# alucas2/raytracing-potato

Measured on AMD Instinct MI355X. Metric: Mrays/s at 1920×1080×256spp bunny scene; 1/2/4/8-GPU scaling + %HBM roofline, higher is better.
Workload: dtype f64

## Files before the change

include/rp_host.h:

```cpp
#ifndef RP_HOST_H
#define RP_HOST_H

#include <stdint.h>

#include "rp.h"

#ifdef __cplusplus
extern "C" {
#endif

typedef struct rph_mesh {
  uint32_t n_vertices, n_indices;
  double* positions;
  double* normals;
  double* uvs;
  uint32_t* indices;
} rph_mesh;

int rph_obj_load(const char* path, rph_mesh* out);
void rph_mesh_free(rph_mesh* m);

int rph_tga_load(const char* path, uint32_t* width, uint32_t* height, uint8_t** rgba);
int rph_tga_save(const char* path, uint32_t width, uint32_t height, const uint8_t* rgba);
void rph_free(void* p);
// ... 28 lines not shown
  uint32_t grid;
  uint64_t n_queue, out_stride;
  uint32_t dv_units[2], dv_tiles_x[2], dv_chunk[2];
} rph_launch_plan;
int rph_plan_launch(uint32_t width, uint32_t height, uint32_t spp, uint32_t max_bounce, uint32_t tile_w, uint32_t tile_h,
                    uint32_t shard, uint32_t num_shards, uint32_t samples_per_stream, uint32_t shard_map, uint32_t n_frames,
                    uint32_t frame_order, uint32_t unit_queues, uint32_t queue_chunk, uint64_t lanes, rph_launch_plan* out);

int rph_draw_round(uint32_t kind, uint32_t ring_blocks, const uint32_t* ring_image, uint32_t pos, double out[3],
                   uint32_t* new_pos, uint32_t* accepted);

int rph_ray_setup(uint32_t node_format, double qbound, const double* rays, uint64_t n, float* out);

int rph_prim_test(uint32_t kind, const double g[9], const double* rays, uint64_t n, double* out);

const char* rph_last_error(void);

#ifdef __cplusplus
}
#endif
#endif
```

raytracing-potato_amd/csrc/rp_device.h:

```cpp
#pragma once
#include <hip/hip_runtime.h>

#include "rp_kernel.h"

#pragma clang fp contract(off)

#include "rp_draw.h"
#include "rp_ray.h"
#include "rp_isect.h"

#if defined(RPK_ABLATE_RNG) || defined(RPK_ABLATE_UV) || defined(RPK_ABLATE_TEX) || defined(RPK_ABLATE_METAL) || \
    defined(RPK_BATCH_LEAF)
#error "result-changing experiment macros are not part of the product kernel"
#endif
#if defined(RPK_NT_STORE) || defined(RPK_NT_ALL) || defined(RPK_NT_TEX) || defined(RPK_NT_OUT) ||           \
    defined(RPK_SLAB_ALIGN) || defined(RPK_SLAB_PAD) || defined(RPK_COLD_SLAB) || defined(RPK_COLD_IN_SLAB) || \
    defined(RPK_W3) || defined(RPK_W4) || defined(RPK_WAVES) || defined(RPK_TRIES_BALL) ||             \
    defined(RPK_NO_SPECULATIVE) || defined(RPK_NODE_BREAK) || defined(RPK_TRIES) || defined(RPK_RING) ||       \
    defined(RPK_RNG_BATCH) || defined(RPK_RNG_CRIT) || defined(RPK_PRIM_BREAK) || defined(RPK_PRIO_TRAV) ||    \
    defined(RPK_PRIO_SHADE) || defined(RPK_PRIO_REFILL) || defined(RPK_SORT_Q) || defined(RPK_WF_REFILL)
#error "experiment macros are not part of the product kernel (tools/build_variant.sh patches a copy instead)"
#endif

namespace rpk {
// ... 123 lines not shown
  }
  return make_uint4(o[0], o[1], o[2], o[3]);
}

RPK_INLINE void seed_key(uint64_t state, uint32_t key[8]) {
#pragma unroll
  for (int c = 0; c < 8; c++) {
    state = state * 6364136223846793005ull + 11634580027462260723ull;
    uint32_t xs = (uint32_t)(((state >> 18) ^ state) >> 27);
    uint32_t rot = (uint32_t)(state >> 59);
    key[c] = (xs >> rot) | (xs << ((32 - rot) & 31));
  }
}

static constexpr uint32_t RING = 8;
static constexpr uint32_t SLAB_KEY = 0, SLAB_RING = 2;
static constexpr uint32_t RNG_CRIT = 2, RNG_BATCH = 48;
static constexpr uint32_t PRIM_BREAK = 12;

template <uint32_t RN>
struct RngT {
  static constexpr uint32_t ring = RN;
  static constexpr uint32_t tail_n = rpd::ring_tail_words(RN) / 4;
  static constexpr uint32_t tail = SLAB_RING + 4 * RN, jit = tail + tail_n, lane_n = jit + 8;
  static_assert(RN > RNG_CRIT && RN <= RING && (RN & (RN - 1)) == 0,
                "ring: a power of two above the critical refill level (a full ring is never refilled), <= RING");
  static_assert(lane_n % 2 == 0, "lane slab stride must be a multiple of 32 B (keystream blocks on whole sectors)");
  uint4* slab;
  uint32_t pos;
  uint32_t* end;
  uint32_t* jtag;
};
template <class Rng>
RPK_INLINE void store_key(Rng& r, const uint32_t k[8]) {
  r.slab[SLAB_KEY] = make_uint4(k[0], k[1], k[2], k[3]);
  r.slab[SLAB_KEY + 1] = make_uint4(k[4], k[5], k[6], k[7]);
}
RPK_INLINE void store_block(uint4* dst, const uint32_t w[16]) {
#pragma unroll
  for (int q = 0; q < 4; q++) {
    dst[q] = make_uint4(w[4 * q], w[4 * q + 1], w[4 * q + 2], w[4 * q + 3]);
  }
}
RPK_INLINE void store_ring_block(uint4* dst, uint4* tail, const uint32_t w[16]) {
  store_block(dst, w);
  if (tail) {
#pragma unroll
    for (uint32_t q = 0; q < rpd::TAIL_WORDS / 4; q++) tail[q] = make_uint4(w[4 * q], w[4 * q + 1], w[4 * q + 2], w[4 * q + 3]);
  }
}
RPK_INLINE void load_block(const uint4* src, uint32_t w[16]) {
#pragma unroll
  for (int q = 0; q < 4; q++) {
    const uint4 v = src[q];
    w[4 * q] = v.x; w[4 * q + 1] = v.y; w[4 * q + 2] = v.z; w[4 * q + 3] = v.w;
  }
}
template <uint32_t RN>
RPK_INLINE uint4* ring_slot(const RngT<RN>& r, uint32_t b) { return r.slab + SLAB_RING + 4 * (b & (RN - 1u)); }
template <uint32_t RN>
RPK_INLINE uint4* ring_tail(uint4* slab, uint32_t b) {
  return RngT<RN>::tail_n != 0 && (b & (RN - 1u)) == 0u ? slab + RngT<RN>::tail : nullptr;
}
template <uint32_t RN>
RPK_INLINE uint4* jit_slot(const RngT<RN>& r, uint32_t b) { return r.slab + RngT<RN>::jit + 4 * (b & 1u); }

RPK_INLINE uint32_t nth_set(uint64_t m, uint32_t n) {
  uint32_t pos = 0;
#pragma unroll
  for (int w = 32; w >= 1; w >>= 1) {
    const uint32_t c = (uint32_t)__popcll(m & ((1ull << w) - 1ull));
    if (n >= c) { n -= c; m >>= w; pos += (uint32_t)w; }
  }
  return pos;
}
static_assert(BLOCK == 64, "rng_refill: a block is one wave, so a lane's slab is the wave's lane index past the first");
template <uint32_t RN>
RPK_INLINE void rng_refill(RngT<RN>& r, bool alive, bool fresh, uint64_t seed, uint32_t s, uint32_t spp) {
  const uint32_t cur = r.pos >> 4, end = *r.end, have = end - cur;
  const uint32_t b1 = (s + 1) >> 2, b2 = b1 + 1;
  const bool j1 = alive && !fresh && 4 * b1 < spp && r.jtag[(b1 & 1u) * BLOCK] != b1;
  const bool j2 = alive && !fresh && 4 * b2 < spp && r.jtag[(b2 & 1u) * BLOCK] != b2;
  const bool crit = alive && (fresh || have <= RNG_CRIT);
  const bool room = alive && (fresh || have < RN || j1 || j2);
  if (__ballot(crit) == 0 && (uint32_t)__popcll(__ballot(room)) < RNG_BATCH) return;
  const bool main = fresh || crit || !(j1 || j2);
  const uint32_t b = fresh ? 0u : (main ? end : (j1 ? b1 : b2));
  const uint32_t end1 = !room ? end : (fresh ? 1u : (main ? end + 1u : end));
  const uint32_t have1 = end1 - (fresh ? 0u : cur);
  const uint32_t want = alive && have1 <= RNG_CRIT ? min(RNG_CRIT + 1u - have1, RN - have1) : 0u;
  const uint64_t m1 = __ballot(want >= 1u), m2 = __ballot(want >= 2u), ex = __ballot(!room);
  const uint32_t lane = __lane_id();
  const uint64_t below = (1ull << lane) - 1ull;
  const uint32_t n1 = (uint32_t)__popcll(m1), nreq = n1 + (uint32_t)__popcll(m2), nex = (uint32_t)__popcll(ex);
  const uint32_t xr = (uint32_t)__popcll(ex & below);
  const bool sec = !room && xr < nreq;
  uint32_t owner = lane, j = 0u;
  if (sec) {
    if (xr < n1) owner = nth_set(m1, xr);
    else { owner = nth_set(m2, xr - n1); j = 1u; }
  }
  const uint32_t slo = __shfl((uint32_t)seed, (int)owner), shi = __shfl((uint32_t)(seed >> 32), (int)owner);
  const uint32_t oend = __shfl(end1, (int)owner);
  const uint32_t served = (uint32_t)(want >= 1u && (uint32_t)__popcll(m1 & below) < nex) +
                          (uint32_t)(want >= 2u && n1 + (uint32_t)__popcll(m2 & below) < nex);
  if (room || sec) {
    DREG(DREG_REFILL)
    uint32_t k[8], w[16];
    seed_key(room ? seed : ((uint64_t)shi << 32 | slo), k);
    if (fresh) {
      DREG(DREG_BEGIN_PIXEL)
      store_key(r, k);
    }
    const uint32_t bb = room ? b : oend + j;
    chacha12(k, bb, w);
    uint4* oslab = r.slab + ((int)owner - (int)lane) * (int)RngT<RN>::lane_n;
    uint4* dst = room && !main ? jit_slot(r, b) : oslab + SLAB_RING + 4u * (bb & (RN - 1u));
    store_ring_block(dst, room && !main ? nullptr : ring_tail<RN>(oslab, bb), w);
    if (fresh) store_block(jit_slot(r, 0), w);
  }
  if (room) {
    if (fresh) {
      r.pos = 0;
      r.jtag[0] = 0;
      r.jtag[BLOCK] = 0xFFFFFFFFu;
    } else if (!main) {
      r.jtag[(b & 1u) * BLOCK] = b;
    }
  }
  if (room || served) *r.end = end1 + served;
  __builtin_amdgcn_fence(__ATOMIC_ACQ_REL, "wavefront");
}

static __device__ __attribute__((noinline, unused)) void gen_block(const uint4* slab, uint32_t b, uint4* dst, uint4* tail) {
  const uint4 a = slab[SLAB_KEY], c = slab[SLAB_KEY + 1];
  const uint32_t k[8] = {a.x, a.y, a.z, a.w, c.x, c.y, c.z, c.w};
  uint32_t w[16];
  chacha12(k, b, w);
  store_ring_block(dst, tail, w);
}

template <uint32_t RN>
RPK_INLINE uint4 rng_jitter(RngT<RN>& r, uint32_t s) {
  const uint32_t b = s >> 2;
  if (r.jtag[(b & 1u) * BLOCK] != b) {
    DREG(DREG_JIT_FALLBACK)
    gen_block(r.slab, b, jit_slot(r, b), nullptr);
    r.jtag[(b & 1u) * BLOCK] = b;
  }
  return jit_slot(r, b)[s & 3u];
}

using rpd::TRIES;
static_assert((RING & (RING - 1)) == 0, "the ring is indexed as 16 * ring words (a power of two)");
typedef uint32_t u32x4_a8 __attribute__((ext_vector_type(4), aligned(8)));
template <uint32_t STRIDE, uint32_t RN>
RPK_INLINE void ring_window(const RngT<RN>& r, uint32_t a, rpd::Try& t) {
  t.w[4] = 0; t.w[5] = 0;
  if constexpr (RngT<RN>::tail_n != 0) {
    const char* p = reinterpret_cast<const char*>(r.slab + SLAB_RING) + 4u * rpd::value_word(a, 0, RN);
    const u32x4_a8 v = *reinterpret_cast<const u32x4_a8*>(p);
    t.w[0] = v.x; t.w[1] = v.y; t.w[2] = v.z; t.w[3] = v.w;
    if (STRIDE == 6u) {
      const uint2 z = *reinterpret_cast<const uint2*>(p + 16);
      t.w[4] = z.x; t.w[5] = z.y;
    }
  } else {
    const uint2* ring = reinterpret_cast<const uint2*>(r.slab + SLAB_RING);
#pragma unroll
    for (uint32_t k = 0; k < STRIDE / 2u; k++) {
      const uint2 v = ring[rpd::value_word(a, k, RN) >> 1];
      t.w[2 * k] = v.x; t.w[2 * k + 1] = v.y;
    }
  }
}
template <uint32_t RN>
RPK_INLINE void ring_ensure(RngT<RN>& r, uint32_t last_blk) {
  while (last_blk >= *r.end) {
    DREG(DREG_RNG_FALLBACK)
    const uint32_t b = *r.end;
    gen_block(r.slab, b, ring_slot(r, b), ring_tail<RN>(r.slab, b));
    *r.end = b + 1;
  }
}
template <uint32_t STRIDE, uint32_t RN>
RPK_INLINE bool ring_round(RngT<RN>& r, uint32_t a, rpd::Draw& q) {
  ring_ensure(r, rpd::round_last_block(a, STRIDE));
  rpd::Try t[TRIES];
#pragma unroll
  for (uint32_t j = 0; j < TRIES; j++) ring_window<STRIDE>(r, a + STRIDE * j, t[j]);
  return rpd::draw_pick(STRIDE, a, t, q, r.pos);
}
template <uint32_t RN>
RPK_INLINE double gen_f64(RngT<RN>& r) {
  ring_ensure(r, r.pos >> 4);
  const uint2 v = reinterpret_cast<const uint2*>(r.slab + SLAB_RING)[rpd::window_word(r.pos, RN) >> 1];
  r.pos += 2;
  return rpd::words_unit(v.x, v.y);
}


typedef rpi::V3 V3;
RPK_INLINE V3 v3(double x, double y, double z) { V3 r; r.x = x; r.y = y; r.z = z; return r; }
RPK_INLINE V3 add(V3 a, V3 b) { return v3(a.x + b.x, a.y + b.y, a.z + b.z); }
RPK_INLINE V3 sub(V3 a, V3 b) { return v3(a.x - b.x, a.y - b.y, a.z - b.z); }
RPK_INLINE V3 mulc(V3 a, V3 b) { return v3(a.x * b.x, a.y * b.y, a.z * b.z); }
RPK_INLINE V3 smul(double s, V3 a) { return v3(s * a.x, s * a.y, s * a.z); }
RPK_INLINE double dot(V3 a, V3 b) { return (a.x * b.x + a.y * b.y) + a.z * b.z; }
RPK_INLINE double norm2(V3 a) { return (a.x * a.x + a.y * a.y) + a.z * a.z; }
RPK_INLINE V3 normalize(V3 a) { double n = sqrt(norm2(a)); return v3(a.x / n, a.y / n, a.z / n); }
RPK_INLINE V3 reflect(V3 i, V3 n) { return sub(i, smul(2.0 * dot(i, n), n)); }
// ... 127 lines not shown
    asm volatile("" : : "v"(g45.x), "v"(g45.y), "v"(g67.x), "v"(g67.y), "v"(g8k.x));
    rpi::sphere_test(g0, g23.y, o, d, tmin, best, [&](double t) {
      best = t; ts.bestp = (int32_t)k; ts.bestm = mat;
    });
  }
}

template <uint32_t NF>
RPK_INLINE void trav_begin(const KScene& S, V3 o, V3 d, double tmin, double tmax, TravState& t) {
  trav_init<NF>(S, tmax, t, d);
  double best = t.best;
  for (uint32_t k = S.always_first; k < S.always_first + S.n_always; k++) prim_test(S, k, o, d, tmin, best, t);
  t.best = best;
}

typedef __attribute__((address_space(3))) uint32_t lds_u32;
typedef __attribute__((address_space(1))) uint32_t glb_u32;
RPK_INLINE glb_u32* spill_ptr(const KScene& S) { return (glb_u32*)S.spill; }
template <bool SPILL>
RPK_INLINE void stk_put(const KScene& S, lds_u32* stk, uint32_t stride, uint32_t spl, uint32_t i, uint32_t v) {
  if (!SPILL || i < S.lds_depth) stk[i * stride] = v;
  else spill_ptr(S)[spl + i - S.lds_depth] = v;
}
template <bool SPILL>
RPK_INLINE uint32_t stk_get(const KScene& S, const lds_u32* stk, uint32_t stride, uint32_t spl, uint32_t i) {
  if (!SPILL || i < S.lds_depth) return stk[i * stride];
  return spill_ptr(S)[spl + i - S.lds_depth];
}

enum : uint32_t { WORK_VISIT = 2, WORK_TEST = 3, WORK_RAY = 16 };

// ... 804 lines not shown
```

raytracing-potato_amd/csrc/rp_host.cpp:

```cpp
#include "../../include/rp_host.h"

#include <algorithm>
#include <cmath>
#include <cstdio>
#include <cstdlib>
#include <cstring>
#include <fstream>
#include <string>
#include <thread>
#include <unordered_map>
#include <vector>

#include "rp_bvh.h"
#include "rp_draw.h"
#include "rp_isect.h"
#include "rp_kernel.h"
#include "rp_ray.h"
#include "rp_schedule.h"

namespace {

thread_local std::string g_err;

int fail(const std::string& m) {
  g_err = m;
  return RP_EINVAL;
}


struct Cursor {
  const char* p;
};
// ... 649 lines not shown

int rph_prim_test(uint32_t kind, const double g[9], const double* rays, uint64_t n, double* out) {
  if ((kind != rpl::PRIM_SPHERE && kind != rpl::PRIM_TRIANGLE) || !g || (n && (!rays || !out)))
    return fail("rph_prim_test: kind 0 (sphere) or 1 (triangle), non-NULL pointers");
  for (uint64_t r = 0; r < n; r++) {
    const double* q = rays + 8 * r;
    double* h = out + 4 * r;
    h[0] = h[1] = h[2] = h[3] = 0.0;
    prim_test(kind, g, {q[0], q[1], q[2]}, {q[3], q[4], q[5]}, q[6], q[7], [&](double t, double u, double v) {
      h[0] = 1.0; h[1] = t; h[2] = u; h[3] = v;
    });
  }
  return RP_OK;
}

int rph_draw_round(uint32_t kind, uint32_t ring_blocks, const uint32_t* ring_image, uint32_t pos, double out[3],
                   uint32_t* new_pos, uint32_t* accepted) {
  if (kind < rpd::DRAW_SPHERE || kind > rpd::DRAW_DISK || (ring_blocks != 4 && ring_blocks != 8) || (pos & 1u) ||
      !ring_image || !out || !new_pos || !accepted)
    return fail("rph_draw_round: kind 1-4, ring_blocks 4 or 8, even pos, non-NULL pointers");
  out[0] = out[1] = out[2] = 0.0;
  if (kind == rpd::DRAW_UNIFORM) {
    const uint32_t* p = ring_image + rpd::window_word(pos, ring_blocks);
    out[0] = rpd::words_unit(p[0], p[1]);
    *new_pos = pos + 2u;
    *accepted = 1u;
    return RP_OK;
  }
  const uint32_t stride = rpd::draw_stride(kind);
  rpd::Try t[rpd::TRIES];
// ... 78 lines not shown
```

raytracing-potato_amd/csrc/rp_kernel.h:

```cpp
#pragma once
#include <stdint.h>

#include "rp_layout.h"

namespace rpk {

struct KScene {
  const void* nodes;
  const rpl::Prim* prims;
  const rpl::PrimRef* prim_refs;
  const double* vnrm;
  const double* vuv;
  const rpl::Material* mats;
  const rpl::Texture* texs;
  const uint32_t* texels;
  rpl::Emit background;
  uint32_t root;
  uint32_t always_first, n_always;
  double qbound;
  uint32_t node_format;
  uint32_t leaf_break;
  uint32_t stack_depth;
  uint32_t lds_depth;
  uint64_t* diag;
  uint32_t* rng_slab;
  uint32_t* spill;
  uint32_t* unit_t0;
};

uint64_t rng_slab_bytes_per_lane(uint32_t node_format);
enum { RENDER_BLOCK = 64 };

enum { DIAG_N = 416, DIAG_DUR = 352, DIAG_DUR_N = 24, DIAG_DUR_LOG0 = 10 };
enum { DIAG_CYC = 320 };
enum {
  DCYC_SURF, DCYC_SPHUV, DCYC_TEXISSUE, DCYC_SCATTER, DCYC_TEXVAL, DCYC_EMIT, DCYC_START_SAMPLE, DCYC_END_SAMPLE,
  DCYC_NEWRAY, DCYC_REFILL, DCYC_NEXT_BOUNCE, DCYC_NODE_LOOP, DCYC_PRIM_LOOP, DCYC_N
};
#ifndef RPK_DIAG_BIN_TICKS
#define RPK_DIAG_BIN_TICKS 1000000
#endif
enum { DIAG_HIST = 64, DIAG_BIN_TICKS = RPK_DIAG_BIN_TICKS };
enum {
  DREG_NODE, DREG_PRIM, DREG_STEP, DREG_SHADE, DREG_SURF, DREG_SPHUV, DREG_TEX, DREG_LAMBERT, DREG_METAL,
  DREG_DIELEC, DREG_LOOP_LAMBERT, DREG_LOOP_METAL, DREG_END_SAMPLE, DREG_END_PIXEL, DREG_START_SAMPLE,
// ... 108 lines not shown
```

raytracing-potato_amd/csrc/rp_kernel.hip:

```cpp
#include "rp_device.h"

#pragma clang fp contract(off)

namespace rpk {

#define RPK_RENDER_ATTR __attribute__((amdgpu_waves_per_eu(4)))
static constexpr int PRIO_TRAV = 2, PRIO_SHADE = 1, PRIO_REFILL = 0;
template <uint32_t NF>
constexpr uint32_t RingFor = NF == rpl::NODES_Q8 ? 4u : RING;

RPK_INLINE bool meas_unit(uint32_t pipj, uint32_t batch) { return ((pipj ^ (pipj >> 16) ^ batch ^ (pipj >> 3)) & 7u) == 0u; }

template <bool PROBE, bool SPILL, uint32_t NF>
__global__ void __launch_bounds__(BLOCK) RPK_RENDER_ATTR render_kernel(const KArgs args) {
  extern __shared__ uint32_t lds_stack[];
  __shared__ unsigned long long blk_ctr[3];
  DIAG(__shared__ unsigned long long wmax[BLOCK / 64][8];
       if (threadIdx.x < BLOCK / 64 * 8) wmax[threadIdx.x / 8][threadIdx.x % 8] = 0;)
  if (threadIdx.x < 3) blk_ctr[threadIdx.x] = 0;
  DIAG(if (threadIdx.x < 2 * DREG_N) g_dreg[threadIdx.x] = 0;)
  DIAG(if (threadIdx.x < DCYC_N) g_dcyc[threadIdx.x] = 0;)
  DIAG(if (!PROBE && threadIdx.x == 0) atomicMax(&kargs()->diag[10], ~(unsigned long long)__builtin_amdgcn_s_memrealtime());)
  __syncthreads();
  lds_u32* stk = (lds_u32*)(lds_stack + threadIdx.x);

  uint64_t n_rays = 0, n_samples = 0, n_pixels = 0;
  DIAG(uint32_t lane_rays = 0;)
  bool overflow = false;
  DIAG(uint64_t ph[5] = {0, 0, 0, 0, 0}; uint64_t iters = 0, active = 0; TravDiag td; uint64_t t_prev = stamp();)
  DIAG(const uint64_t t_blk = __builtin_amdgcn_s_memrealtime(); uint64_t t_pix = t_blk, t_retire = t_blk; uint32_t rays_pix = 0;
       auto tbin = [&](uint64_t t) { return (uint32_t)min<uint64_t>((t - t_blk) / DIAG_BIN_TICKS, DIAG_HIST - 1); };)

  __shared__ double c_sum[3 * BLOCK];
  __shared__ double c_T[3 * BLOCK];
  __shared__ uint32_t c_u[8 * BLOCK];
  const uint32_t tid = threadIdx.x;
  uint32_t& slot = c_u[tid];
  uint32_t& pipj = c_u[BLOCK + tid];
  uint32_t& s = c_u[3 * BLOCK + tid];
  uint32_t& hits = c_u[4 * BLOCK + tid];
  uint32_t& batch = c_u[2 * BLOCK + tid];
  double& sum_x = c_sum[tid];
  double& sum_y = c_sum[BLOCK + tid];
  double& sum_z = c_sum[2 * BLOCK + tid];
  double& T_x = c_T[tid];
  double& T_y = c_T[BLOCK + tid];
  double& T_z = c_T[2 * BLOCK + tid];
  uint32_t depth = 0;
  uint32_t work = 0;
  bool first = true;
  RngT<RingFor<NF>> rng;
  rng.slab = reinterpret_cast<uint4*>(kargs()->S.rng_slab) + ((uint64_t)blockIdx.x * BLOCK + tid) * RngT<RingFor<NF>>::lane_n;
  rng.end = c_u + 5 * BLOCK + tid;
  rng.jtag = c_u + 6 * BLOCK + tid;
  rng.pos = 0;
  V3 o = v3(0, 0, 0), d = v3(0, 0, 1);
  T_x = T_y = T_z = 1.0;
  s = 0;
  hits = 0;
  sum_x = sum_y = sum_z = 0.0;
  TravState ts;
  ts.cur = rpl::ENTRY_EMPTY;
  ts.leaf = 0u;
  ts.sp = 0u;
  ts.best = 0.0;
  ts.bestp = -1;
  ts.bestm = KM_UNKNOWN;
  ts.bu = ts.bv = 0.0;
  ts.gy = ts.py = 0u;
// ... 566 lines not shown
  if (pos >= n) return;
  const uint32_t r = pos % N, k = pos / N, t = plan ? plan[pos] : pos;
  fcost[t] = sum[r * rank_stride + k];
  fcost[TILE_SORT_MAX + t] = mx[r * rank_stride + k];
}

int launch_learn_costs(const uint32_t* sum, const uint32_t* max, uint32_t rank_stride, uint32_t nranks, uint32_t n_tiles,
                       const uint32_t* plan, uint32_t* fcost, void* stream) {
  if (n_tiles == 0 || n_tiles > TILE_SORT_MAX || nranks == 0) return (int)hipErrorInvalidValue;
  hipLaunchKernelGGL(learn_costs_kernel, dim3((n_tiles + 255) / 256), dim3(256), 0, (hipStream_t)stream, sum, max,
                     rank_stride, nranks, n_tiles, plan, fcost);
  return (int)hipGetLastError();
}

uint64_t rng_slab_bytes_per_lane(uint32_t nf) {
  const uint32_t n = nf == rpl::NODES_Q8   ? RngT<RingFor<rpl::NODES_Q8>>::lane_n
                     : nf == rpl::NODES_W8 ? RngT<RingFor<rpl::NODES_W8>>::lane_n
                                           : RngT<RingFor<rpl::NODES_F32>>::lane_n;
  return (uint64_t)n * sizeof(uint4);
}

int render_blocks_per_cu(uint32_t lds_depth, bool spill, uint32_t nf, int* blocks) {
  const size_t lds = (size_t)lds_depth * BLOCK * sizeof(uint32_t);
  if (nf == rpl::NODES_W8) {
    if (spill) return (int)hipOccupancyMaxActiveBlocksPerMultiprocessor(blocks, render_kernel<false, true, rpl::NODES_W8>, BLOCK, lds);
    return (int)hipOccupancyMaxActiveBlocksPerMultiprocessor(blocks, render_kernel<false, false, rpl::NODES_W8>, BLOCK, lds);
  }
  if (nf == rpl::NODES_Q8) {
    if (spill) return (int)hipOccupancyMaxActiveBlocksPerMultiprocessor(blocks, render_kernel<false, true, rpl::NODES_Q8>, BLOCK, lds);
    return (int)hipOccupancyMaxActiveBlocksPerMultiprocessor(blocks, render_kernel<false, false, rpl::NODES_Q8>, BLOCK, lds);
  }
  if (spill) return (int)hipOccupancyMaxActiveBlocksPerMultiprocessor(blocks, render_kernel<false, true, rpl::NODES_F32>, BLOCK, lds);
  return (int)hipOccupancyMaxActiveBlocksPerMultiprocessor(blocks, render_kernel<false, false, rpl::NODES_F32>, BLOCK, lds);
}
// ... 20 lines not shown
```

raytracing-potato_amd/csrc/rp_scene.cpp:

```cpp
#include <chrono>
#include <cmath>

#include "rp_bvh.h"
#include "rp_state.h"

static_assert(rpk::CTR_N == RP_COUNTERS_LEN, "kernel counter block = the ABI's");
static_assert(rpk::CTR_RAYS == RP_CTR_RAYS && rpk::CTR_STATUS == RP_CTR_STATUS, "counter order");
static_assert(rpk::STATUS_STACK_OVERFLOW == RP_STATUS_STACK_OVERFLOW && rpk::STATUS_PLAN_MISMATCH == RP_STATUS_PLAN_MISMATCH,
              "status bits");
static_assert(sizeof(rp_render_params) == 48, "rp_render_params layout (bindings mirror it)");

__attribute__((visibility("hidden"))) thread_local std::string g_err;

namespace {

template <class T, class U>
int upload(const std::vector<T>& v, DevBuf<U>& out) {
  hipError_t e;
  if (!out.alloc((v.empty() ? 1 : v.size()) * (sizeof(T) / sizeof(U)), &e))
    return fail(RP_ENOMEM, std::string("hipMalloc: ") + hipGetErrorString(e));
  if (!v.empty()) {
    e = hipMemcpy(out.get(), v.data(), sizeof(T) * v.size(), hipMemcpyHostToDevice);
    if (e != hipSuccess) return fail(RP_EHIP, std::string("hipMemcpy: ") + hipGetErrorString(e));
  }
// ... 193 lines not shown
    return rc;
  if (!s->d_diag.alloc(rpk::DIAG_N) || hipMemset(s->d_diag.get(), 0, sizeof(uint64_t) * rpk::DIAG_N) != hipSuccess)
    return fail(RP_ENOMEM, "hipMalloc diagnostics");
  s->ks.diag = s->d_diag.get();
  s->ks.nodes = s->d_nodes.get(), s->ks.prims = s->d_prims.get(), s->ks.prim_refs = s->d_prim_refs.get();
  s->ks.vnrm = s->d_vnrm.get(), s->ks.vuv = s->d_vuv.get();
  s->ks.mats = s->d_mats.get(), s->ks.texs = s->d_texs.get(), s->ks.texels = s->d_texels.get();
  s->ks.background = ps.background;
  s->ks.root = ps.root;
  s->ks.always_first = ps.always_first;
  s->ks.n_always = ps.n_always;
  s->ks.qbound = ps.qbound;
  s->ks.node_format = node_format;
  s->ks.stack_depth = 3 * ps.max_depth + 4 + 3;
  if (node_format == rpl::NODES_W8) s->ks.stack_depth = 4 * (ps.max_depth + 1) + 3;
  if (s->ks.stack_depth < 17) s->ks.stack_depth = 17;
  const bool debug_stack = opt.debug_stack_depth != 0;
  if (debug_stack) s->ks.stack_depth = opt.debug_stack_depth;
  s->n_nodes = n_tree_nodes;
  s->n_leaves = ps.n_leaves;
  s->n_prims = desc->n_hittables;
  s->max_depth = ps.max_depth;
  s->device_bytes = rp_node_bytes(node_format) * n_tree_nodes + (sizeof(rpl::Prim) + sizeof(rpl::PrimRef)) * n_tree_prims +
                    sizeof(double) * 5 * n_vert + sizeof(rpl::Material) * ps.materials.size() +
                    sizeof(rpl::Texture) * ps.textures.size() + sizeof(uint32_t) * ps.texels.size();
  s->tiles_auto = RP_TILES_COST;
  s->ks.leaf_break = opt.leaf_break ? opt.leaf_break : (s->device_bytes > (256ull << 20) ? 16u : 8u);
  if (s->opt.trav_threshold == 0) s->opt.trav_threshold = s->device_bytes > (256ull << 20) ? 32u : DEF_TRAV_THRESHOLD;
  s->ks.lds_depth = s->ks.stack_depth;
  int bpc = 0;
  if (rpk::render_blocks_per_cu(s->ks.stack_depth, false, node_format, &bpc) != 0 || bpc < 1) bpc = 1;
  int bpc_spill = 0;
  if (!debug_stack && rpk::render_blocks_per_cu(17, true, node_format, &bpc_spill) == 0 && bpc_spill > bpc) {
    uint32_t L = s->ks.stack_depth - 1;
    int b = 0;
    while (L > 17 && (rpk::render_blocks_per_cu(L, true, node_format, &b) != 0 || b < bpc_spill)) L--;
    s->ks.lds_depth = L;
    bpc = bpc_spill;
  }
  if (!debug_stack && opt.lds_depth && opt.lds_depth < s->ks.stack_depth) {
    s->ks.lds_depth = opt.lds_depth;
    if (rpk::render_blocks_per_cu(opt.lds_depth, true, node_format, &bpc) != 0 || bpc < 1) bpc = 1;
  }
  s->blocks_per_cu = bpc;
  phase[4] = lap();
  if ((rc = ws_alloc(s.get(), &s->ws0))) return rc;
  phase[5] = lap();
  std::memcpy(s->build_s, phase, sizeof phase);
  *out = s.release();
  return RP_OK;
}
// ... 95 lines not shown
```

raytracing-potato_amd/rtpotato/_ffi.py:

```python
from __future__ import annotations

import ctypes
import os
from ctypes import (POINTER, Structure, c_char_p, c_double, c_float, c_int, c_int64, c_uint8, c_uint32,
                    c_uint64, c_void_p)

PKG_DIR = os.path.dirname(os.path.dirname(os.path.abspath(__file__)))
LIB_DIR = os.path.join(PKG_DIR, "lib")

RP_OK, RP_EINVAL, RP_EHIP, RP_ENOMEM, RP_ENODEV, RP_EINTERNAL, RP_ERCCL = 0, -1, -2, -3, -4, -5, -6
RP_HITTABLE_SPHERE, RP_HITTABLE_TRIANGLE = 0, 1
RP_SCATTER_NONE, RP_SCATTER_LAMBERT, RP_SCATTER_METAL, RP_SCATTER_DIELECTRIC = 0, 1, 2, 3
RP_ABSORB_BLACK_BODY, RP_ABSORB_WHITE_BODY, RP_ABSORB_ALBEDO, RP_ABSORB_ALBEDO_MAP = 0, 1, 2, 3
(RP_EMIT_NONE, RP_EMIT_DEBUG_NORMALS, RP_EMIT_COLOR, RP_EMIT_SKY_GRADIENT, RP_EMIT_SKY_SPHERE) = range(5)
(RP_TEXTURE_MISSING, RP_TEXTURE_DEBUG_UVS, RP_TEXTURE_SOLID, RP_TEXTURE_IMAGE, RP_TEXTURE_CHECKER,
 RP_TEXTURE_NOISE, RP_TEXTURE_PERLIN) = range(7)
RP_ROOT_BVH, RP_ROOT_LIST = 0, 1
RP_COUNTERS_LEN = 4
RP_SAMPLES_PER_STREAM = 32
RP_COMM_ID_BYTES = 128
RP_BUILDER_AUTO, RP_BUILDER_HOST, RP_BUILDER_DEVICE, RP_BUILDER_PLOC = 0, 1, 2, 3
RP_NODES_AUTO, RP_NODES_F32, RP_NODES_Q8, RP_NODES_W8 = 0, 1, 2, 3
RP_TILES_AUTO, RP_TILES_PLAIN, RP_TILES_COST, RP_TILES_MORTON, RP_TILES_PROBE = 0, 1, 2, 3, 4
RP_QUEUES_AUTO, RP_QUEUES_SINGLE, RP_QUEUES_XCD_TILES, RP_QUEUES_XCD_REGIONS = 0, 1, 2, 3
# ... 102 lines not shown
              "rp_render_multi", "rp_shard_unpack_map", "rp_workspace_tile_map", "rp_frame_assemble_ws", "rp_build_id",
              "rp_workspace_tile_costs", "rp_workspace_set_tile_costs", "rp_scene_build_times",
              "rp_workspace_frame_info", "rp_workspace_reserve_frames", "rp_render_frames_device_ws", "rp_frames_gather",
              "rp_workspace_unit_order", "rp_frames_block_words", "rp_frames_pack", "rp_frames_unpack",
              "rp_render_aov_device_ws", "rp_render_aov"]
class rph_launch_plan(Structure):
    _fields_ = [("n_shard_tiles", c_uint32), ("nbatch", c_uint32), ("plan_block", c_uint32), ("n_slots", c_uint64),
                ("gather_stride", c_uint64), ("block_words", c_uint64), ("queue_groups", c_uint32),
                ("queue_chunk", c_uint32), ("frames_inter", c_uint32), ("sortable", c_uint32), ("measure", c_uint32),
                ("grid", c_uint32), ("n_queue", c_uint64), ("out_stride", c_uint64), ("dv_units", c_uint32 * 2),
                ("dv_tiles_x", c_uint32 * 2), ("dv_chunk", c_uint32 * 2)]


HOST_SYMBOLS = ["rph_obj_load", "rph_mesh_free", "rph_tga_load", "rph_tga_save", "rph_free", "rph_to_srgb_u8",
                "rph_lookat", "rph_sky_panorama", "rph_bvh_selfcheck", "rph_bvh_traversal_stats", "rph_bvh_selfcheck_ex", "rph_bvh_traversal_stats_ex", "rph_bvh_tree_hash", "rph_last_error",
                "rph_stdrng_u64", "rph_make_div32", "rph_plan_launch", "rph_draw_round", "rph_ray_setup", "rph_prim_test"]


def rp_lib_path() -> str:
    return os.path.join(LIB_DIR, "librp.so")


def host_lib_path() -> str:
    return os.path.join(LIB_DIR, "librp_host.so")


def rp() -> ctypes.CDLL:
    global _rp
    if _rp is not None:
        return _rp
    path = os.environ.get("RP_LIB") or rp_lib_path()
# ... 98 lines not shown
    lib.rph_lookat.argtypes = [c_double * 3, c_double * 3, c_double * 3, c_double * 9]
    lib.rph_lookat.restype = None
    lib.rph_sky_panorama.argtypes = [c_uint32, c_uint32, c_void_p]
    lib.rph_bvh_selfcheck.argtypes = [POINTER(rp_scene_desc), c_uint32, POINTER(c_uint64)]
    lib.rph_bvh_traversal_stats.argtypes = [POINTER(rp_scene_desc), c_void_p, c_uint64, c_uint32, c_void_p]
    lib.rph_bvh_selfcheck_ex.argtypes = [POINTER(rp_scene_desc), c_uint32, c_uint32, POINTER(c_uint64)]
    lib.rph_bvh_traversal_stats_ex.argtypes = [POINTER(rp_scene_desc), c_void_p, c_uint64, c_uint32, c_uint32, c_void_p]
    lib.rph_bvh_tree_hash.argtypes = [POINTER(rp_scene_desc), c_uint32, c_uint32, POINTER(c_uint64)]
    lib.rph_last_error.restype = c_char_p
    lib.rph_stdrng_u64.argtypes = [c_void_p, c_uint64, c_uint64, c_void_p]
    lib.rph_make_div32.argtypes = [c_uint32, POINTER(c_uint32), POINTER(c_uint32)]
    lib.rph_draw_round.argtypes = [c_uint32, c_uint32, c_void_p, c_uint32, c_void_p, POINTER(c_uint32),
                                   POINTER(c_uint32)]
    lib.rph_ray_setup.argtypes = [c_uint32, c_double, c_void_p, c_uint64, c_void_p]
    lib.rph_prim_test.argtypes = [c_uint32, c_void_p, c_void_p, c_uint64, c_void_p]
    lib.rph_plan_launch.argtypes = [c_uint32] * 14 + [c_uint64, POINTER(rph_launch_plan)]
    _host = lib
    return lib


def check(code: int, lib: ctypes.CDLL | None = None) -> None:
    if code != RP_OK:
        lib = lib or rp()
        fn = lib.rp_last_error if hasattr(lib, "rp_last_error") else lib.rph_last_error
        raise RPError(code, (fn() or b"").decode(errors="replace"))


def check_host(code: int) -> None:
    if code != RP_OK:
        raise RPError(code, (host().rph_last_error() or b"").decode(errors="replace"))
# ... 4 lines not shown
```

Baseline: 7654.

## Keep per-lane ChaCha keys in LDS and route refill owners through LDS table

For non-Q8 node formats, each lane's ChaCha key is computed once per pixel and kept in shared memory instead of the global RNG slab. Secondary lanes that refill on another lane's behalf now read the owner's key from LDS rather than shuffling its seed and re-running seed_key. The owner-to-executor mapping is built through an LDS request table instead of the nth_set bit search. The RNG slab per lane shrinks by 32 B and the stack-depth LDS floor is lowered to offset the extra shared arrays. The cost is about 2.1 KB more LDS per block, which could lower occupancy or shrink the LDS traversal stack.

Result: no change. 7690 (median of 6 runs) (+0.5%).

```diff
diff --git a/include/rp_host.h b/include/rp_host.h
--- a/include/rp_host.h
+++ b/include/rp_host.h
@@ -66,6 +66,9 @@
 
 int rph_prim_test(uint32_t kind, const double g[9], const double* rays, uint64_t n, double* out);
 
+int rph_refill_assign(const uint8_t room[64], const uint8_t want[64], uint32_t owner[64], uint32_t block[64],
+                      uint32_t served[64]);
+
 const char* rph_last_error(void);
 
 #ifdef __cplusplus
diff --git a/raytracing-potato_amd/csrc/rp_device.h b/raytracing-potato_amd/csrc/rp_device.h
--- a/raytracing-potato_amd/csrc/rp_device.h
+++ b/raytracing-potato_amd/csrc/rp_device.h
@@ -6,6 +6,7 @@
 #pragma clang fp contract(off)
 
 #include "rp_draw.h"
+#include "rp_refill.h"
 #include "rp_ray.h"
 #include "rp_isect.h"
 
@@ -161,15 +162,18 @@
 }
 
 static constexpr uint32_t RING = 8;
-static constexpr uint32_t SLAB_KEY = 0, SLAB_RING = 2;
+typedef __attribute__((address_space(3))) uint32_t lds_u32;
+typedef __attribute__((address_space(3))) uint8_t lds_u8;
 static constexpr uint32_t RNG_CRIT = 2, RNG_BATCH = 48;
 static constexpr uint32_t PRIM_BREAK = 12;
 
-template <uint32_t RN>
+template <uint32_t RN, bool KL>
 struct RngT {
   static constexpr uint32_t ring = RN;
+  static constexpr bool key_lds = KL;
+  static constexpr uint32_t ring0 = KL ? 0u : 2u;
   static constexpr uint32_t tail_n = rpd::ring_tail_words(RN) / 4;
-  static constexpr uint32_t tail = SLAB_RING + 4 * RN, jit = tail + tail_n, lane_n = jit + 8;
+  static constexpr uint32_t tail = ring0 + 4 * RN, jit = tail + tail_n, lane_n = jit + 8;
   static_assert(RN > RNG_CRIT && RN <= RING && (RN & (RN - 1)) == 0,
                 "ring: a power of two above the critical refill level (a full ring is never refilled), <= RING");
   static_assert(lane_n % 2 == 0, "lane slab stride must be a multiple of 32 B (keystream blocks on whole sectors)");
@@ -177,11 +181,12 @@
   uint32_t pos;
   uint32_t* end;
   uint32_t* jtag;
+  lds_u32* key;
+  lds_u8* req;
 };
-template <class Rng>
-RPK_INLINE void store_key(Rng& r, const uint32_t k[8]) {
-  r.slab[SLAB_KEY] = make_uint4(k[0], k[1], k[2], k[3]);
-  r.slab[SLAB_KEY + 1] = make_uint4(k[4], k[5], k[6], k[7]);
+RPK_INLINE void load_key(const lds_u32* col, uint32_t k[8]) {
+#pragma unroll
+  for (int w = 0; w < 8; w++) k[w] = col[w * BLOCK];
 }
 RPK_INLINE void store_block(uint4* dst, const uint32_t w[16]) {
 #pragma unroll
@@ -203,27 +208,19 @@
     w[4 * q] = v.x; w[4 * q + 1] = v.y; w[4 * q + 2] = v.z; w[4 * q + 3] = v.w;
   }
 }
-template <uint32_t RN>
-RPK_INLINE uint4* ring_slot(const RngT<RN>& r, uint32_t b) { return r.slab + SLAB_RING + 4 * (b & (RN - 1u)); }
-template <uint32_t RN>
+template <uint32_t RN, bool KL>
+RPK_INLINE uint4* ring_slot(const RngT<RN, KL>& r, uint32_t b) { return r.slab + RngT<RN, KL>::ring0 + 4 * (b & (RN - 1u)); }
+template <uint32_t RN, bool KL>
 RPK_INLINE uint4* ring_tail(uint4* slab, uint32_t b) {
-  return RngT<RN>::tail_n != 0 && (b & (RN - 1u)) == 0u ? slab + RngT<RN>::tail : nullptr;
-}
-template <uint32_t RN>
-RPK_INLINE uint4* jit_slot(const RngT<RN>& r, uint32_t b) { return r.slab + RngT<RN>::jit + 4 * (b & 1u); }
-
-RPK_INLINE uint32_t nth_set(uint64_t m, uint32_t n) {
-  uint32_t pos = 0;
-#pragma unroll
-  for (int w = 32; w >= 1; w >>= 1) {
-    const uint32_t c = (uint32_t)__popcll(m & ((1ull << w) - 1ull));
-    if (n >= c) { n -= c; m >>= w; pos += (uint32_t)w; }
-  }
-  return pos;
-}
-static_assert(BLOCK == 64, "rng_refill: a block is one wave, so a lane's slab is the wave's lane index past the first");
-template <uint32_t RN>
-RPK_INLINE void rng_refill(RngT<RN>& r, bool alive, bool fresh, uint64_t seed, uint32_t s, uint32_t spp) {
+  return RngT<RN, KL>::tail_n != 0 && (b & (RN - 1u)) == 0u ? slab + RngT<RN, KL>::tail : nullptr;
+}
+template <uint32_t RN, bool KL>
+RPK_INLINE uint4* jit_slot(const RngT<RN, KL>& r, uint32_t b) { return r.slab + RngT<RN, KL>::jit + 4 * (b & 1u); }
+
+static_assert(BLOCK == 64 && rpf::LANES == 64,
+              "rng_refill: a block is one wave, so a lane's slab, key column and hand-off byte are indexed by the wave's lane");
+template <uint32_t RN, bool KL>
+RPK_INLINE void rng_refill(RngT<RN, KL>& r, bool alive, bool fresh, uint64_t seed, uint32_t s, uint32_t spp) {
   const uint32_t cur = r.pos >> 4, end = *r.end, have = end - cur;
   const uint32_t b1 = (s + 1) >> 2, b2 = b1 + 1;
   const bool j1 = alive && !fresh && 4 * b1 < spp && r.jtag[(b1 & 1u) * BLOCK] != b1;
@@ -235,35 +232,54 @@
   const uint32_t b = fresh ? 0u : (main ? end : (j1 ? b1 : b2));
   const uint32_t end1 = !room ? end : (fresh ? 1u : (main ? end + 1u : end));
   const uint32_t have1 = end1 - (fresh ? 0u : cur);
-  const uint32_t want = alive && have1 <= RNG_CRIT ? min(RNG_CRIT + 1u - have1, RN - have1) : 0u;
-  const uint64_t m1 = __ballot(want >= 1u), m2 = __ballot(want >= 2u), ex = __ballot(!room);
+  const uint32_t want = alive ? rpf::want_blocks(have1, RNG_CRIT, RN) : 0u;
+  const rpf::Pass ps = rpf::make_pass(__ballot(want >= 1u), __ballot(want >= 2u), __ballot(!room));
   const uint32_t lane = __lane_id();
-  const uint64_t below = (1ull << lane) - 1ull;
-  const uint32_t n1 = (uint32_t)__popcll(m1), nreq = n1 + (uint32_t)__popcll(m2), nex = (uint32_t)__popcll(ex);
-  const uint32_t xr = (uint32_t)__popcll(ex & below);
-  const bool sec = !room && xr < nreq;
+  const uint32_t q1 = rpf::request_index(ps, lane, 0u), q2 = rpf::request_index(ps, lane, 1u);
+  if (want >= 1u && rpf::request_served(ps, q1)) r.req[q1] = (uint8_t)lane;
+  if (want >= 2u && rpf::request_served(ps, q2)) r.req[q2] = (uint8_t)lane;
+  const uint32_t served = rpf::served(ps, lane, want);
+  if (room) *r.end = end1;
+  if (fresh) {
+    DREG(DREG_BEGIN_PIXEL)
+    if constexpr (KL) {
+      uint32_t k[8];
+      seed_key(seed, k);
+#pragma unroll
+      for (int w = 0; w < 8; w++) r.key[w * BLOCK] = k[w];
+    }
+  }
+  __builtin_amdgcn_fence(__ATOMIC_ACQ_REL, "wavefront");
+  const uint32_t xr = rpf::executor_rank(ps, lane);
+  const bool sec = !room && rpf::executor_busy(ps, xr);
   uint32_t owner = lane, j = 0u;
   if (sec) {
-    if (xr < n1) owner = nth_set(m1, xr);
-    else { owner = nth_set(m2, xr - n1); j = 1u; }
-  }
-  const uint32_t slo = __shfl((uint32_t)seed, (int)owner), shi = __shfl((uint32_t)(seed >> 32), (int)owner);
-  const uint32_t oend = __shfl(end1, (int)owner);
-  const uint32_t served = (uint32_t)(want >= 1u && (uint32_t)__popcll(m1 & below) < nex) +
-                          (uint32_t)(want >= 2u && n1 + (uint32_t)__popcll(m2 & below) < nex);
+    owner = r.req[xr];
+    j = rpf::executor_block(ps, xr);
+  }
+  uint32_t slo = 0u, shi = 0u;
+  if constexpr (!KL) {
+    slo = __shfl((uint32_t)seed, (int)owner);
+    shi = __shfl((uint32_t)(seed >> 32), (int)owner);
+  }
   if (room || sec) {
     DREG(DREG_REFILL)
     uint32_t k[8], w[16];
-    seed_key(room ? seed : ((uint64_t)shi << 32 | slo), k);
-    if (fresh) {
-      DREG(DREG_BEGIN_PIXEL)
-      store_key(r, k);
+    const uint32_t oend = r.end[(int)owner - (int)lane];
+    if constexpr (KL) {
+      load_key(r.key + ((int)owner - (int)lane), k);
+    } else {
+      seed_key(room ? seed : ((uint64_t)shi << 32 | slo), k);
+      if (fresh) {
+        r.slab[0] = make_uint4(k[0], k[1], k[2], k[3]);
+        r.slab[1] = make_uint4(k[4], k[5], k[6], k[7]);
+      }
     }
     const uint32_t bb = room ? b : oend + j;
     chacha12(k, bb, w);
-    uint4* oslab = r.slab + ((int)owner - (int)lane) * (int)RngT<RN>::lane_n;
-    uint4* dst = room && !main ? jit_slot(r, b) : oslab + SLAB_RING + 4u * (bb & (RN - 1u));
-    store_ring_block(dst, room && !main ? nullptr : ring_tail<RN>(oslab, bb), w);
+    uint4* oslab = r.slab + ((int)owner - (int)lane) * (int)RngT<RN, KL>::lane_n;
+    uint4* dst = room && !main ? jit_slot(r, b) : oslab + RngT<RN, KL>::ring0 + 4u * (bb & (RN - 1u));
+    store_ring_block(dst, room && !main ? nullptr : ring_tail<RN, KL>(oslab, bb), w);
     if (fresh) store_block(jit_slot(r, 0), w);
   }
   if (room) {
@@ -275,24 +291,35 @@
       r.jtag[(b & 1u) * BLOCK] = b;
     }
   }
-  if (room || served) *r.end = end1 + served;
+  if (served) *r.end = end1 + served;
   __builtin_amdgcn_fence(__ATOMIC_ACQ_REL, "wavefront");
 }
 
-static __device__ __attribute__((noinline, unused)) void gen_block(const uint4* slab, uint32_t b, uint4* dst, uint4* tail) {
-  const uint4 a = slab[SLAB_KEY], c = slab[SLAB_KEY + 1];
+static __device__ __attribute__((noinline, unused)) void gen_block(const lds_u32* key, uint32_t b, uint4* dst, uint4* tail) {
+  uint32_t k[8], w[16];
+  load_key(key, k);
+  chacha12(k, b, w);
+  store_ring_block(dst, tail, w);
+}
+
+static __device__ __attribute__((noinline, unused)) void gen_block_slab(const uint4* slab, uint32_t b, uint4* dst, uint4* tail) {
+  const uint4 a = slab[0], c = slab[1];
   const uint32_t k[8] = {a.x, a.y, a.z, a.w, c.x, c.y, c.z, c.w};
   uint32_t w[16];
   chacha12(k, b, w);
   store_ring_block(dst, tail, w);
 }
-
-template <uint32_t RN>
-RPK_INLINE uint4 rng_jitter(RngT<RN>& r, uint32_t s) {
+template <uint32_t RN, bool KL>
+RPK_INLINE void gen_lane_block(const RngT<RN, KL>& r, uint32_t b, uint4* dst, uint4* tail) {
+  if constexpr (KL) gen_block(r.key, b, dst, tail);
+  else gen_block_slab(r.slab, b, dst, tail);
+}
+template <uint32_t RN, bool KL>
+RPK_INLINE uint4 rng_jitter(RngT<RN, KL>& r, uint32_t s) {
   const uint32_t b = s >> 2;
   if (r.jtag[(b & 1u) * BLOCK] != b) {
     DREG(DREG_JIT_FALLBACK)
-    gen_block(r.slab, b, jit_slot(r, b), nullptr);
+    gen_lane_block(r, b, jit_slot(r, b), nullptr);
     r.jtag[(b & 1u) * BLOCK] = b;
   }
   return jit_slot(r, b)[s & 3u];
@@ -301,11 +328,11 @@
 using rpd::TRIES;
 static_assert((RING & (RING - 1)) == 0, "the ring is indexed as 16 * ring words (a power of two)");
 typedef uint32_t u32x4_a8 __attribute__((ext_vector_type(4), aligned(8)));
-template <uint32_t STRIDE, uint32_t RN>
-RPK_INLINE void ring_window(const RngT<RN>& r, uint32_t a, rpd::Try& t) {
+template <uint32_t STRIDE, uint32_t RN, bool KL>
+RPK_INLINE void ring_window(const RngT<RN, KL>& r, uint32_t a, rpd::Try& t) {
   t.w[4] = 0; t.w[5] = 0;
-  if constexpr (RngT<RN>::tail_n != 0) {
-    const char* p = reinterpret_cast<const char*>(r.slab + SLAB_RING) + 4u * rpd::value_word(a, 0, RN);
+  if constexpr (RngT<RN, KL>::tail_n != 0) {
+    const char* p = reinterpret_cast<const char*>(r.slab + RngT<RN, KL>::ring0) + 4u * rpd::value_word(a, 0, RN);
     const u32x4_a8 v = *reinterpret_cast<const u32x4_a8*>(p);
     t.w[0] = v.x; t.w[1] = v.y; t.w[2] = v.z; t.w[3] = v.w;
     if (STRIDE == 6u) {
@@ -313,7 +340,7 @@
       t.w[4] = z.x; t.w[5] = z.y;
     }
   } else {
-    const uint2* ring = reinterpret_cast<const uint2*>(r.slab + SLAB_RING);
+    const uint2* ring = reinterpret_cast<const uint2*>(r.slab + RngT<RN, KL>::ring0);
 #pragma unroll
     for (uint32_t k = 0; k < STRIDE / 2u; k++) {
       const uint2 v = ring[rpd::value_word(a, k, RN) >> 1];
@@ -321,27 +348,27 @@
     }
   }
 }
-template <uint32_t RN>
-RPK_INLINE void ring_ensure(RngT<RN>& r, uint32_t last_blk) {
+template <uint32_t RN, bool KL>
+RPK_INLINE void ring_ensure(RngT<RN, KL>& r, uint32_t last_blk) {
   while (last_blk >= *r.end) {
     DREG(DREG_RNG_FALLBACK)
     const uint32_t b = *r.end;
-    gen_block(r.slab, b, ring_slot(r, b), ring_tail<RN>(r.slab, b));
+    gen_lane_block(r, b, ring_slot(r, b), ring_tail<RN, KL>(r.slab, b));
     *r.end = b + 1;
   }
 }
-template <uint32_t STRIDE, uint32_t RN>
-RPK_INLINE bool ring_round(RngT<RN>& r, uint32_t a, rpd::Draw& q) {
+template <uint32_t STRIDE, uint32_t RN, bool KL>
+RPK_INLINE bool ring_round(RngT<RN, KL>& r, uint32_t a, rpd::Draw& q) {
   ring_ensure(r, rpd::round_last_block(a, STRIDE));
   rpd::Try t[TRIES];
 #pragma unroll
   for (uint32_t j = 0; j < TRIES; j++) ring_window<STRIDE>(r, a + STRIDE * j, t[j]);
   return rpd::draw_pick(STRIDE, a, t, q, r.pos);
 }
-template <uint32_t RN>
-RPK_INLINE double gen_f64(RngT<RN>& r) {
+template <uint32_t RN, bool KL>
+RPK_INLINE double gen_f64(RngT<RN, KL>& r) {
   ring_ensure(r, r.pos >> 4);
-  const uint2 v = reinterpret_cast<const uint2*>(r.slab + SLAB_RING)[rpd::window_word(r.pos, RN) >> 1];
+  const uint2 v = reinterpret_cast<const uint2*>(r.slab + RngT<RN, KL>::ring0)[rpd::window_word(r.pos, RN) >> 1];
   r.pos += 2;
   return rpd::words_unit(v.x, v.y);
 }
@@ -499,7 +526,6 @@
   t.best = best;
 }
 
-typedef __attribute__((address_space(3))) uint32_t lds_u32;
 typedef __attribute__((address_space(1))) uint32_t glb_u32;
 RPK_INLINE glb_u32* spill_ptr(const KScene& S) { return (glb_u32*)S.spill; }
 template <bool SPILL>
diff --git a/raytracing-potato_amd/csrc/rp_host.cpp b/raytracing-potato_amd/csrc/rp_host.cpp
--- a/raytracing-potato_amd/csrc/rp_host.cpp
+++ b/raytracing-potato_amd/csrc/rp_host.cpp
@@ -16,6 +16,7 @@
 #include "rp_isect.h"
 #include "rp_kernel.h"
 #include "rp_ray.h"
+#include "rp_refill.h"
 #include "rp_schedule.h"
 
 namespace {
@@ -695,6 +696,35 @@
   return RP_OK;
 }
 
+int rph_refill_assign(const uint8_t room[64], const uint8_t want[64], uint32_t owner[64], uint32_t block[64],
+                      uint32_t served[64]) {
+  if (!room || !want || !owner || !block || !served) return fail("rph_refill_assign: non-NULL pointers");
+  uint64_t m1 = 0, m2 = 0, ex = 0;
+  for (uint32_t l = 0; l < rpf::LANES; l++) {
+    if (want[l] > 2u || (want[l] && !room[l])) return fail("rph_refill_assign: want 0-2, and only of a lane with room");
+    m1 |= (uint64_t)(want[l] >= 1u) << l;
+    m2 |= (uint64_t)(want[l] >= 2u) << l;
+    ex |= (uint64_t)(!room[l]) << l;
+  }
+  const rpf::Pass ps = rpf::make_pass(m1, m2, ex);
+  uint8_t table[rpf::LANES];
+  std::memset(table, (int)rpf::NO_OWNER, sizeof table);
+  for (uint32_t l = 0; l < rpf::LANES; l++) {
+    for (uint32_t second = 0; second < want[l]; second++) {
+      const uint32_t q = rpf::request_index(ps, l, second);
+      if (rpf::request_served(ps, q)) table[q] = (uint8_t)l;
+    }
+    served[l] = rpf::served(ps, l, want[l]);
+  }
+  for (uint32_t l = 0; l < rpf::LANES; l++) {
+    const uint32_t x = rpf::executor_rank(ps, l);
+    const bool sec = !room[l] && rpf::executor_busy(ps, x);
+    owner[l] = sec ? table[x] : 0xFFFFFFFFu;
+    block[l] = sec ? rpf::executor_block(ps, x) : 0u;
+  }
+  return RP_OK;
+}
+
 int rph_draw_round(uint32_t kind, uint32_t ring_blocks, const uint32_t* ring_image, uint32_t pos, double out[3],
                    uint32_t* new_pos, uint32_t* accepted) {
   if (kind < rpd::DRAW_SPHERE || kind > rpd::DRAW_DISK || (ring_blocks != 4 && ring_blocks != 8) || (pos & 1u) ||
diff --git a/raytracing-potato_amd/csrc/rp_kernel.h b/raytracing-potato_amd/csrc/rp_kernel.h
--- a/raytracing-potato_amd/csrc/rp_kernel.h
+++ b/raytracing-potato_amd/csrc/rp_kernel.h
@@ -29,6 +29,7 @@
 };
 
 uint64_t rng_slab_bytes_per_lane(uint32_t node_format);
+uint32_t render_lds_floor(uint32_t node_format);
 enum { RENDER_BLOCK = 64 };
 
 enum { DIAG_N = 416, DIAG_DUR = 352, DIAG_DUR_N = 24, DIAG_DUR_LOG0 = 10 };
diff --git a/raytracing-potato_amd/csrc/rp_kernel.hip b/raytracing-potato_amd/csrc/rp_kernel.hip
--- a/raytracing-potato_amd/csrc/rp_kernel.hip
+++ b/raytracing-potato_amd/csrc/rp_kernel.hip
@@ -8,6 +8,10 @@
 static constexpr int PRIO_TRAV = 2, PRIO_SHADE = 1, PRIO_REFILL = 0;
 template <uint32_t NF>
 constexpr uint32_t RingFor = NF == rpl::NODES_Q8 ? 4u : RING;
+template <uint32_t NF>
+constexpr bool KeyInLds = NF != rpl::NODES_Q8;
+template <uint32_t NF>
+using RngFor = RngT<RingFor<NF>, KeyInLds<NF>>;
 
 RPK_INLINE bool meas_unit(uint32_t pipj, uint32_t batch) { return ((pipj ^ (pipj >> 16) ^ batch ^ (pipj >> 3)) & 7u) == 0u; }
 
@@ -34,6 +38,8 @@
   __shared__ double c_sum[3 * BLOCK];
   __shared__ double c_T[3 * BLOCK];
   __shared__ uint32_t c_u[8 * BLOCK];
+  __shared__ uint32_t c_key[8 * BLOCK];
+  __shared__ uint8_t c_req[BLOCK];
   const uint32_t tid = threadIdx.x;
   uint32_t& slot = c_u[tid];
   uint32_t& pipj = c_u[BLOCK + tid];
@@ -49,10 +55,12 @@
   uint32_t depth = 0;
   uint32_t work = 0;
   bool first = true;
-  RngT<RingFor<NF>> rng;
-  rng.slab = reinterpret_cast<uint4*>(kargs()->S.rng_slab) + ((uint64_t)blockIdx.x * BLOCK + tid) * RngT<RingFor<NF>>::lane_n;
+  RngFor<NF> rng;
+  rng.slab = reinterpret_cast<uint4*>(kargs()->S.rng_slab) + ((uint64_t)blockIdx.x * BLOCK + tid) * RngFor<NF>::lane_n;
   rng.end = c_u + 5 * BLOCK + tid;
   rng.jtag = c_u + 6 * BLOCK + tid;
+  rng.key = (lds_u32*)c_key + tid;
+  rng.req = (lds_u8*)c_req;
   rng.pos = 0;
   V3 o = v3(0, 0, 0), d = v3(0, 0, 1);
   T_x = T_y = T_z = 1.0;
@@ -649,10 +657,15 @@
 }
 
 uint64_t rng_slab_bytes_per_lane(uint32_t nf) {
-  const uint32_t n = nf == rpl::NODES_Q8   ? RngT<RingFor<rpl::NODES_Q8>>::lane_n
-                     : nf == rpl::NODES_W8 ? RngT<RingFor<rpl::NODES_W8>>::lane_n
-                                           : RngT<RingFor<rpl::NODES_F32>>::lane_n;
+  const uint32_t n = nf == rpl::NODES_Q8   ? RngFor<rpl::NODES_Q8>::lane_n
+                     : nf == rpl::NODES_W8 ? RngFor<rpl::NODES_W8>::lane_n
+                                           : RngFor<rpl::NODES_F32>::lane_n;
   return (uint64_t)n * sizeof(uint4);
+}
+
+uint32_t render_lds_floor(uint32_t nf) {
+  const bool kl = nf == rpl::NODES_Q8 ? KeyInLds<rpl::NODES_Q8> : nf == rpl::NODES_W8 ? KeyInLds<rpl::NODES_W8> : KeyInLds<rpl::NODES_F32>;
+  return kl ? 11u : 17u;
 }
 
 int render_blocks_per_cu(uint32_t lds_depth, bool spill, uint32_t nf, int* blocks) {
diff --git a/raytracing-potato_amd/csrc/rp_refill.h b/raytracing-potato_amd/csrc/rp_refill.h
--- /dev/null
+++ b/raytracing-potato_amd/csrc/rp_refill.h
@@ -0,0 +1,50 @@
+#pragma once
+#include <stdint.h>
+
+#if defined(__HIPCC__)
+#define RPF_FN __host__ __device__ __forceinline__
+#else
+#define RPF_FN inline
+#endif
+
+namespace rpf {
+
+static constexpr uint32_t LANES = 64;
+static constexpr uint32_t NO_OWNER = 0xFFu;
+
+RPF_FN uint32_t popc(uint64_t m) { return (uint32_t)__builtin_popcountll(m); }
+RPF_FN uint64_t below(uint32_t lane) { return (1ull << lane) - 1ull; }
+
+struct Pass {
+  uint64_t m1, m2, ex;
+  uint32_t n1, nreq, nex;
+};
+RPF_FN Pass make_pass(uint64_t m1, uint64_t m2, uint64_t ex) {
+  Pass p;
+  p.m1 = m1; p.m2 = m2; p.ex = ex;
+  p.n1 = popc(m1);
+  p.nreq = p.n1 + popc(m2);
+  p.nex = popc(ex);
+  return p;
+}
+
+RPF_FN uint32_t want_blocks(uint32_t have1, uint32_t crit, uint32_t rn) {
+  if (have1 > crit) return 0u;
+  const uint32_t a = crit + 1u - have1, b = rn - have1;
+  return a < b ? a : b;
+}
+
+RPF_FN uint32_t request_index(const Pass& p, uint32_t lane, uint32_t second) {
+  return second ? p.n1 + popc(p.m2 & below(lane)) : popc(p.m1 & below(lane));
+}
+RPF_FN bool request_served(const Pass& p, uint32_t q) { return q < p.nex; }
+RPF_FN uint32_t served(const Pass& p, uint32_t lane, uint32_t want) {
+  return (uint32_t)(want >= 1u && request_served(p, request_index(p, lane, 0u))) +
+         (uint32_t)(want >= 2u && request_served(p, request_index(p, lane, 1u)));
+}
+
+RPF_FN uint32_t executor_rank(const Pass& p, uint32_t lane) { return popc(p.ex & below(lane)); }
+RPF_FN bool executor_busy(const Pass& p, uint32_t x) { return x < p.nreq; }
+RPF_FN uint32_t executor_block(const Pass& p, uint32_t x) { return x >= p.n1 ? 1u : 0u; }
+
+}
diff --git a/raytracing-potato_amd/csrc/rp_scene.cpp b/raytracing-potato_amd/csrc/rp_scene.cpp
--- a/raytracing-potato_amd/csrc/rp_scene.cpp
+++ b/raytracing-potato_amd/csrc/rp_scene.cpp
@@ -231,7 +231,8 @@
   s->ks.node_format = node_format;
   s->ks.stack_depth = 3 * ps.max_depth + 4 + 3;
   if (node_format == rpl::NODES_W8) s->ks.stack_depth = 4 * (ps.max_depth + 1) + 3;
-  if (s->ks.stack_depth < 17) s->ks.stack_depth = 17;
+  const uint32_t LDS_FLOOR = rpk::render_lds_floor(node_format);
+  if (s->ks.stack_depth < LDS_FLOOR) s->ks.stack_depth = LDS_FLOOR;
   const bool debug_stack = opt.debug_stack_depth != 0;
   if (debug_stack) s->ks.stack_depth = opt.debug_stack_depth;
   s->n_nodes = n_tree_nodes;
@@ -248,10 +249,10 @@
   int bpc = 0;
   if (rpk::render_blocks_per_cu(s->ks.stack_depth, false, node_format, &bpc) != 0 || bpc < 1) bpc = 1;
   int bpc_spill = 0;
-  if (!debug_stack && rpk::render_blocks_per_cu(17, true, node_format, &bpc_spill) == 0 && bpc_spill > bpc) {
+  if (!debug_stack && rpk::render_blocks_per_cu(LDS_FLOOR, true, node_format, &bpc_spill) == 0 && bpc_spill > bpc) {
     uint32_t L = s->ks.stack_depth - 1;
     int b = 0;
-    while (L > 17 && (rpk::render_blocks_per_cu(L, true, node_format, &b) != 0 || b < bpc_spill)) L--;
+    while (L > LDS_FLOOR && (rpk::render_blocks_per_cu(L, true, node_format, &b) != 0 || b < bpc_spill)) L--;
     s->ks.lds_depth = L;
     bpc = bpc_spill;
   }
diff --git a/raytracing-potato_amd/rtpotato/_ffi.py b/raytracing-potato_amd/rtpotato/_ffi.py
--- a/raytracing-potato_amd/rtpotato/_ffi.py
+++ b/raytracing-potato_amd/rtpotato/_ffi.py
@@ -140,7 +140,8 @@
 
 HOST_SYMBOLS = ["rph_obj_load", "rph_mesh_free", "rph_tga_load", "rph_tga_save", "rph_free", "rph_to_srgb_u8",
                 "rph_lookat", "rph_sky_panorama", "rph_bvh_selfcheck", "rph_bvh_traversal_stats", "rph_bvh_selfcheck_ex", "rph_bvh_traversal_stats_ex", "rph_bvh_tree_hash", "rph_last_error",
-                "rph_stdrng_u64", "rph_make_div32", "rph_plan_launch", "rph_draw_round", "rph_ray_setup", "rph_prim_test"]
+                "rph_stdrng_u64", "rph_make_div32", "rph_plan_launch", "rph_draw_round", "rph_ray_setup", "rph_prim_test",
+                "rph_refill_assign"]
 
 
 def rp_lib_path() -> str:
@@ -269,6 +270,7 @@
                                    POINTER(c_uint32)]
     lib.rph_ray_setup.argtypes = [c_uint32, c_double, c_void_p, c_uint64, c_void_p]
     lib.rph_prim_test.argtypes = [c_uint32, c_void_p, c_void_p, c_uint64, c_void_p]
+    lib.rph_refill_assign.argtypes = [c_void_p] * 5
     lib.rph_plan_launch.argtypes = [c_uint32] * 14 + [c_uint64, POINTER(rph_launch_plan)]
     _host = lib
     return lib
```
